# crowsonkb/k-diffusion

Measured on AMD Instinct MI355X. Metric: images/sec, 256x256 image_transformer_v2, 50-step DPM++2M (whole job), higher is better.
Workload: dtype f32

## Files before the change

k-diffusion_amd/csrc/gemm_x3.hip:

```cpp
#include "x3_common.h"

namespace kd {
namespace x3 {

struct XArgs {
  const float* A; const char* Wp; float* C;
  b16::u16* Cl; int c_split;
  const float* scale; int scale_stride, rows_per_sample; float eps;
  int M, N, n_tiles, n_splits;
  int n_heads; const float* qk_scale; const float* pos; const float* freq; int qkv_packed;
  float out_add;
  const float* sigma; float sigma_data; int gh, gw, chan;
  const float* R;
  int warm;
  unsigned long long* clk;
};

template <int NC , int EPI>
__global__ __launch_bounds__(256, NC <= 8 ? 2 : 1) void gemm_x3_astat_kernel(const XArgs p) {
  constexpr int K = NC * 16, NK = NC / 2;
  constexpr int NSTG = NC <= 8 ? 4 : 8, PDIST = NSTG - 1, PB = 4;
  constexpr bool GEGLU = EPI == KD_EPI_GEGLU;
  constexpr int NCOL = GEGLU ? 64 : 128;
  constexpr int NST = GEGLU ? 8 : 16;
  constexpr int WAREA = (NSTG / 4) * STG;
  constexpr int KH = WAREA / 128 >= K ? K : WAREA / 128;
  constexpr bool AG = NC >= 32;
  constexpr int NR = K / KH, CPR = KH / 4;
  constexpr int PIECES = 32 * CPR / 64;
  constexpr int SCL = K * 4 < 1024 ? 1024 : K * 4;
  static_assert(NK % NSTG == 0 || NSTG % NK == 0, "ring slot of a stage must be a compile-time constant");
  static_assert(CPR >= 16 && NC % NR == 0, "source-side chunk swizzle spans 16 chunk positions");
  extern __shared__ __attribute__((aligned(16))) char smem[];
  const int tid = threadIdx.x, lane = tid & 63, l31 = lane & 31, lh = lane >> 5;
  const int wid = __builtin_amdgcn_readfirstlane(tid >> 6);
  const auto warm = code_warm_begin<(NC <= 8 ? 14 : 24) * 1024>((int)blockIdx.x < p.warm && tid < 64);
  const PanelSplit ps = panel_split(p.n_splits, p.n_tiles);
  const int nt_begin = ps.t_begin, n_tiles = ps.t_end - ps.t_begin, total = n_tiles * NK;
  const int m0 = ps.panel * 128;
  const bool probe = p.clk && blockIdx.x == 0 && tid == 0;
  if (probe) { p.clk[0] = __builtin_amdgcn_s_memtime(); p.clk[1] = __builtin_amdgcn_s_memrealtime(); }
  const WgStamp wgs = wg_stamp_begin(p.clk);

  f32x16 acc[4];
  if constexpr (EPI == KD_EPI_RESIDUAL) {
    const int rrow = min(m0 + wid * 32 + l31, p.M - 1);
    const float* rp = p.R + (size_t)rrow * p.N + nt_begin * NCOL + 4 * lh;
#pragma unroll
    for (int j = 0; j < 4; ++j)
#pragma unroll
      for (int g = 0; g < 4; ++g) {
        const f32x4 v = *reinterpret_cast<const f32x4*>(rp + 32 * j + 8 * g);
#pragma unroll
        for (int e = 0; e < 4; ++e) acc[j][4 * g + e] = v[e];
      }
  }

  const char* wp = p.Wp + (size_t)nt_begin * NK * STG + wid * (PB * 1024) + lane * 16;
  auto issue_piece = [&](int s_, int j) {
    const int s = min(s_, total - 1);
    const char* src = wp + (size_t)s * STG;
    char* dst = smem + (s_ % NSTG) * STG + wid * (PB * 1024);
    __builtin_amdgcn_global_load_lds((const __attribute__((address_space(1))) void*)(src + j * 1024),
                                     (__attribute__((address_space(3))) void*)(dst + j * 1024), 16, 0, 0);
  };
  auto issue = [&](int s_) {
#pragma unroll
    for (int j = 0; j < PB; ++j) issue_piece(s_, j);
  };

  const int row = m0 + wid * 32 + l31;
  const bool ok = row < p.M;
  const int rowc = ok ? row : p.M - 1;
  bf16x8 a_hi[AG ? 1 : NC], a_lo[AG ? 1 : NC];
  float rs;
  {
    char* stage = smem + wid * WAREA;
    char* scl = smem + NSTG * STG + wid * SCL;
    const int r_first = min(m0 + wid * 32, p.M - 1), r_last = min(m0 + wid * 32 + 31, p.M - 1);
    constexpr bool nrm = EPI != KD_EPI_RESIDUAL;
    const bool uni = nrm && (p.scale_stride == 0 || r_first / p.rows_per_sample == r_last / p.rows_per_sample);
    if (uni) {
      const char* ssrc = reinterpret_cast<const char*>(p.scale + (size_t)(r_first / p.rows_per_sample) * p.scale_stride);
#pragma unroll
      for (int i = 0; i < SCL / 1024; ++i)
        __builtin_amdgcn_global_load_lds((const __attribute__((address_space(1))) void*)(ssrc + (i * 1024 + lane * 16) % (K * 4)),
                                         (__attribute__((address_space(3))) void*)(scl + i * 1024), 16, 0, 0);
    }
    const float* sp = p.scale + (size_t)(rowc / p.rows_per_sample) * p.scale_stride + 8 * lh;
    const float* spl = reinterpret_cast<const float*>(scl) + 8 * lh;
    float ssq = 0.f;
    static_for<NR>([&](auto r_) {
      constexpr int r = decltype(r_)::value;
#pragma unroll
      for (int i = 0; i < PIECES; ++i) {
        const int ci = i * 64 + lane, rr = ci / CPR, qs = ci % CPR;
        const int grow = min(m0 + wid * 32 + rr, p.M - 1);
        const char* src = reinterpret_cast<const char*>(p.A + (size_t)grow * K + r * KH) + ((qs ^ (rr & 15)) << 4);
        __builtin_amdgcn_global_load_lds((const __attribute__((address_space(1))) void*)src,
                                         (__attribute__((address_space(3))) void*)(stage + i * 1024), 16, 0, 0);
      }
// ... 20 lines not shown
        __builtin_amdgcn_sched_barrier(0);
        static_for<4>([&](auto u_) {
          constexpr int u = decltype(u_)::value;
#pragma unroll
          for (int e = 0; e < 4; ++e) ssq = fmaf(x0[u][e], x0[u][e], fmaf(x1[u][e], x1[u][e], ssq));
          u32x4 hi, lo;
          if constexpr (nrm) split8(x0[u] * s0[u], x1[u] * s1[u], hi, lo);
          else split8(x0[u], x1[u], hi, lo);
          if constexpr (AG) {
            areg_write4<8 * (c0 + u)>(hi);
            areg_write4<8 * (c0 + u) + 4>(lo);
          } else {
            asm volatile("" : "+v"(hi), "+v"(lo));
            a_hi[c0 + u] = __builtin_bit_cast(bf16x8, hi);
            a_lo[c0 + u] = __builtin_bit_cast(bf16x8, lo);
          }
        });
        __builtin_amdgcn_sched_barrier(0);
      });
      if constexpr (NR > 1) asm volatile("s_waitcnt lgkmcnt(0)" ::: "memory");
    });
    ssq += __shfl_xor(ssq, 32, 64);
    rs = nrm ? rsqrtf(ssq / (float)K + p.eps) : 1.f;
  }
  float py = 0.f, px = 0.f;
  if (EPI == KD_EPI_QKV) {
    qk_tab_fill(reinterpret_cast<float*>(smem + NSTG * STG + 4 * SCL + 4 * 2048), tid, p);
    token_pos(p.pos, rowc % p.rows_per_sample, py, px);
  }
  code_warm_end(warm);
  asm volatile("s_waitcnt vmcnt(0) lgkmcnt(0)" ::: "memory");
  KD_BARRIER();
  const bool full_panel = m0 + 128 <= p.M;
#pragma unroll
  for (int s = 0; s < PDIST; ++s) issue(s);
  if (probe) p.clk[4] = __builtin_amdgcn_s_memtime();

  const int o0 = swz64(l31, lh), o1 = swz64(l31, 2 + lh);
  char* strip = smem + NSTG * STG + 4 * SCL + wid * 2048;
  const char* qkc = smem + NSTG * STG + 4 * SCL + 4 * 2048;
  float* st_row[2];
  bool st_ok[2];
#pragma unroll
  for (int it = 0; it < 2; ++it) {
    const int r = m0 + wid * 32 + 16 * it + (lane >> 2);
    st_ok[it] = r < p.M;
    st_row[it] = p.C + (size_t)min(r, p.M - 1) * p.N + 4 * (lane & 3);
  }
  if constexpr (EPI != KD_EPI_RESIDUAL) {
#pragma unroll
    for (int j = 0; j < 4; ++j)
#pragma unroll
      for (int r = 0; r < 16; ++r) acc[j][r] = 0.f;
  }
  if constexpr (AG) asm volatile("s_nop 3" : "+v"(acc[0]), "+v"(acc[1]), "+v"(acc[2]), "+v"(acc[3]));

  bf16x8 wh[2][4], wl[2][4];
  int ou0[2] = {0, 0}, ou1[2] = {0, 0};
  if constexpr (EPI == KD_EPI_UNPATCH_NCHW) {
#pragma unroll
    for (int j = 0; j < 2; ++j) {
      const int np = 32 * j + l31, q = np >> 2, py = q / p.chan, cch = q - py * p.chan;
      const int n = np < 16 * p.chan ? (py * 4 + (np & 3)) * p.chan + cch : np;
      ou0[j] = swz64(n, lh);
      ou1[j] = swz64(n, 2 + lh);
    }
  }
  auto read_frags = [&](int slot, int h, bf16x8 (&fh)[4], bf16x8 (&fl)[4]) {
    if constexpr (EPI == KD_EPI_UNPATCH_NCHW) {
#pragma unroll
      for (int j = 0; j < 2; ++j) {
        const char* st = smem + slot * STG + (h ? ou1[j] : ou0[j]);
        fh[j] = *reinterpret_cast<const bf16x8*>(st);
        fl[j] = *reinterpret_cast<const bf16x8*>(st + IMG);
      }
    } else {
      const char* st = smem + slot * STG + (h ? o1 : o0);
#pragma unroll
      for (int j = 0; j < 4; ++j) {
        fh[j] = *reinterpret_cast<const bf16x8*>(st + j * 32 * 64);
        fl[j] = *reinterpret_cast<const bf16x8*>(st + IMG + j * 32 * 64);
      }
    }
  };
  wait_vm(PB * (PDIST - 1));
  KD_BARRIER();
  read_frags(0, 0, wh[0], wl[0]);

  for (int nt = 0; nt < n_tiles; ++nt) {
    static_for<NK>([&](auto ks_) {
      constexpr int ks = decltype(ks_)::value;
      const int s = nt * NK + ks;
      auto mm = [&](auto b_, int j, bool w_lo, auto a_lo_) {
        constexpr int b = decltype(b_)::value, al = decltype(a_lo_)::value, c = 2 * ks + b;
        if (EPI == KD_EPI_UNPATCH_NCHW && j >= 2) return;
        const bf16x8& w = w_lo ? wl[b][j] : wh[b][j];
        if constexpr (AG) mfma_ag<8 * c + 4 * al>(acc[j], w);
        else mfma_a(acc[j], w, al ? a_lo[c] : a_hi[c]);
      };
      constexpr std::integral_constant<int, 0> I0{};
      constexpr std::integral_constant<int, 1> I1{};
      if constexpr (AG) {
        mm(I0, 0, true, I0);
        __builtin_amdgcn_sched_barrier(0);
        read_frags(ks % NSTG, 1, wh[1], wl[1]);
        __builtin_amdgcn_sched_barrier(0);
#pragma unroll
        for (int j = 1; j < 4; ++j) mm(I0, j, true, I0);
      } else {
        read_frags(ks % NSTG, 1, wh[1], wl[1]);
#pragma unroll
        for (int j = 0; j < 4; ++j) mm(I0, j, true, I0);
      }
#pragma unroll
      for (int j = 0; j < 4; ++j) mm(I0, j, false, I1);
#pragma unroll
      for (int j = 0; j < 4; ++j) mm(I0, j, false, I0);
      if constexpr (!AG) {
        __builtin_amdgcn_sched_group_barrier(0x008, 1, 0);
        __builtin_amdgcn_sched_group_barrier(0x100, 8, 0);
        __builtin_amdgcn_sched_group_barrier(0x008, 11, 0);
      }
      __builtin_amdgcn_sched_barrier(0);
      {
        int allow = PB * (PDIST - 2);
        if (full_panel && nt > 0 && ks + 2 <= PDIST) allow += NST;
        wait_vm(allow);
        KD_BARRIER();
      }
      mm(I1, 0, true, I0);
      if constexpr (AG) __builtin_amdgcn_sched_barrier(0);
      read_frags((ks + 1) % NSTG, 0, wh[0], wl[0]);
      if constexpr (!AG) {
        __builtin_amdgcn_sched_group_barrier(0x008, 1, 0);
        __builtin_amdgcn_sched_group_barrier(0x100, 8, 0);
      }
      __builtin_amdgcn_sched_barrier(0);
      mm(I1, 1, true, I0);
      mm(I1, 2, true, I0);
      issue_piece(s + PDIST, 0);
      __builtin_amdgcn_sched_barrier(0);
      mm(I1, 3, true, I0);
      mm(I1, 0, false, I1);
      mm(I1, 1, false, I1);
      issue_piece(s + PDIST, 1);
      __builtin_amdgcn_sched_barrier(0);
      mm(I1, 2, false, I1);
      mm(I1, 3, false, I1);
      mm(I1, 0, false, I0);
      issue_piece(s + PDIST, 2);
      __builtin_amdgcn_sched_barrier(0);
      mm(I1, 1, false, I0);
      mm(I1, 2, false, I0);
      issue_piece(s + PDIST, 3);
      mm(I1, 3, false, I0);
      __builtin_amdgcn_sched_barrier(0);
    });
    if constexpr (AG) asm volatile("s_nop 15\n\ts_nop 3" : "+v"(acc[0]), "+v"(acc[1]), "+v"(acc[2]), "+v"(acc[3]));
    if (probe && nt == 0) p.clk[5] = __builtin_amdgcn_s_memtime();

    const int n0 = (nt_begin + nt) * NCOL;
    auto store_block = [&](const f32x4 (&v)[4], int col) {
#pragma unroll
      for (int hb = 0; hb < 2; ++hb) {
#pragma unroll
        for (int gg = 0; gg < 2; ++gg)
          *reinterpret_cast<f32x4*>(strip + l31 * 64 + (((2 * gg + lh) ^ ((l31 >> 2) & 1)) << 4)) = v[2 * hb + gg];
#pragma unroll
        for (int it = 0; it < 2; ++it) {
          const int r16 = 16 * it + (lane >> 2), c = lane & 3;
          const f32x4 o = *reinterpret_cast<const f32x4*>(strip + r16 * 64 + ((c ^ ((r16 >> 2) & 1)) << 4));
          if (st_ok[it]) st16(st_row[it] + col + 16 * hb, o);
        }
      }
    };
    if (GEGLU) {
      const float rsh = 0.5f * rs;
#pragma unroll
      for (int jj = 0; jj < 2; ++jj) {
        f32x4 blk[4];
#pragma unroll
        for (int g = 0; g < 4; ++g) {
          const f32x2 a = geglu_pair(f32x2{acc[2 * jj][4 * g], acc[2 * jj][4 * g + 1]} * rsh, f32x2{acc[2 * jj + 1][4 * g], acc[2 * jj + 1][4 * g + 1]} * rs);
          const f32x2 b = geglu_pair(f32x2{acc[2 * jj][4 * g + 2], acc[2 * jj][4 * g + 3]} * rsh, f32x2{acc[2 * jj + 1][4 * g + 2], acc[2 * jj + 1][4 * g + 3]} * rs);
          blk[g] = f32x4{a.x, a.y, b.x, b.y};
        }
        if (p.c_split) {
          float v[16], hi[16], lo[16];
#pragma unroll
          for (int g = 0; g < 4; ++g)
#pragma unroll
            for (int q = 0; q < 4; ++q) v[4 * g + q] = blk[g][q];
#pragma unroll
          for (int r = 0; r < 16; r += 2) {
            const unsigned h = pack_bf16(v[r], v[r + 1]);
            hi[r] = b16::bf_lo(h);
            hi[r + 1] = b16::bf_hi(h);
            lo[r] = v[r] - hi[r];
            lo[r + 1] = v[r + 1] - hi[r + 1];
          }
          const size_t off = (size_t)rowc * p.N + n0 + 32 * jj;
          b16::store_block_bf16(reinterpret_cast<b16::u16*>(p.C) + off, hi, lh, ok);
          b16::store_block_bf16(p.Cl + off, lo, lh, ok);
        } else {
          store_block(blk, n0 + 32 * jj);
        }
      }
    } else if (EPI == KD_EPI_QKV) {
#pragma unroll
      for (int vv = 0; vv < 2; ++vv) {
        const int vec = (n0 >> 6) + vv;
        const int which = vec >= 2 * p.n_heads ? 2 : (vec >= p.n_heads ? 1 : 0), head = vec - which * p.n_heads;
        f32x16& a0 = acc[2 * vv];
        f32x16& a1 = acc[2 * vv + 1];
        if (which < 2) {
          qk_prep_head(qkc, head, lh, a0, a1, rs, p.eps, py, px);
        } else {
#pragma unroll
          for (int r = 0; r < 16; ++r) { a0[r] *= rs; a1[r] *= rs; }
        }
#pragma unroll
        for (int jj = 0; jj < 2; ++jj) {
          f32x4 blk[4];
          const f32x16& a = jj ? a1 : a0;
          if (p.qkv_packed) {
#pragma unroll
            for (int g = 0; g < 4; ++g) blk[g] = pack_split4(f32x4{a[4 * g], a[4 * g + 1], a[4 * g + 2], a[4 * g + 3]});
          } else {
#pragma unroll
            for (int g = 0; g < 4; ++g) blk[g] = f32x4{a[4 * g], a[4 * g + 1], a[4 * g + 2], a[4 * g + 3]};
          }
          store_block(blk, n0 + 64 * vv + 32 * jj);
        }
      }
    } else if (EPI == KD_EPI_UNPATCH_NCHW) {
      const int per = p.gh * p.gw, bb = rowc / per, rr = rowc - bb * per, ty = rr / p.gw, tx = rr - ty * p.gw;
      float c_out = 1.f, c_skip = 0.f;
      if (p.sigma) {
        const float sg = p.sigma[bb], sd = p.sigma_data, var = sg * sg + sd * sd;
        c_skip = sd * sd / var;
        c_out = sg * sd / sqrtf(var);
      }
      const int Himg = 4 * p.gh, Wimg = 4 * p.gw;
#pragma unroll
      for (int j = 0; j < 2; ++j)
#pragma unroll
        for (int g = 0; g < 4; ++g) {
          const int q = 8 * j + 2 * g + lh, py = q / p.chan, cch = q - py * p.chan;
          if (q < 4 * p.chan && ok) {
            const size_t o = (((size_t)bb * p.chan + cch) * Himg + 4 * ty + py) * Wimg + 4 * tx;
            f32x4 v = f32x4{acc[j][4 * g], acc[j][4 * g + 1], acc[j][4 * g + 2], acc[j][4 * g + 3]} * (rs * c_out);
            if (p.sigma) v = v + *reinterpret_cast<const f32x4*>(p.R + o) * c_skip;
            st16(p.C + o, v);
          }
        }
    } else {
#pragma unroll
      for (int j = 0; j < 4; ++j) {
        f32x4 blk[4];
#pragma unroll
        for (int g = 0; g < 4; ++g) blk[g] = f32x4{acc[j][4 * g], acc[j][4 * g + 1], acc[j][4 * g + 2], acc[j][4 * g + 3]} * rs + p.out_add;
        store_block(blk, n0 + 32 * j);
      }
    }
    if (probe && nt == 0) p.clk[6] = __builtin_amdgcn_s_memtime();
#pragma unroll
    for (int j = 0; j < 4; ++j)
#pragma unroll
      for (int r = 0; r < 16; ++r) acc[j][r] = 0.f;
    if constexpr (AG) asm volatile("s_nop 3" : "+v"(acc[0]), "+v"(acc[1]), "+v"(acc[2]), "+v"(acc[3]));
  }
  asm volatile("s_waitcnt vmcnt(0)" ::: "memory");
  if (probe) { p.clk[2] = __builtin_amdgcn_s_memtime(); p.clk[3] = __builtin_amdgcn_s_memrealtime(); p.clk[7] = (unsigned long long)total; }
  wg_stamp_end(wgs);
}

template <int EPI>
__global__ __launch_bounds__(256, 2) void gemm_x3h_kernel(const XArgs p) {
  constexpr int NC = 16, K = 256, NK = 8;
  constexpr int NSTG = 4, PDIST = NSTG - 1, PB = 4, UNIT = 4;
  constexpr bool GEGLU = EPI == KD_EPI_GEGLU;
  constexpr int HCOL = GEGLU ? 32 : 64;
  constexpr int NST = GEGLU ? 4 : 8;
  constexpr int KH = 128, NR = K / KH, CPR = KH / 4, PIECES = 32 * CPR / 64, SCL = 1024, SUB = 8192, HALF = 4096, CB = 2;
  extern __shared__ __attribute__((aligned(16))) char smem[];
  const int tid = threadIdx.x, lane = tid & 63, l31 = lane & 31, lh = lane >> 5;
  const int wid = __builtin_amdgcn_readfirstlane(tid >> 6);
  const auto warm = code_warm_begin<20 * 1024>((int)blockIdx.x < p.warm && tid < 64);
  const PanelSplit ps = panel_split(p.n_splits, p.n_tiles);
  const int ht_begin = ps.t_begin, n_ht = ps.t_end - ps.t_begin, total = n_ht * UNIT;
  const int m0 = ps.panel * 128;
  const bool probe = p.clk && blockIdx.x == (gridDim.x * 5) / 8 && tid == 0;
  if (probe) { p.clk[0] = __builtin_amdgcn_s_memtime(); p.clk[1] = __builtin_amdgcn_s_memrealtime(); }
  const WgStamp wgs = wg_stamp_begin(p.clk);

  const char* wp = p.Wp + wid * 1024 + lane * 16;
  auto issue_piece = [&](int q_, int j) {
    const int q = min(q_, total - 1), ht = ht_begin + (q >> 2), u = q & 3;
    const char* src = wp + ((size_t)(ht >> 1) * NK + 2 * u + (j >> 1)) * STG + (j & 1) * IMG + (ht & 1) * HALF;
    char* dst = smem + (q_ % NSTG) * STG + (j >> 1) * SUB + (j & 1) * HALF + wid * 1024;
    __builtin_amdgcn_global_load_lds((const __attribute__((address_space(1))) void*)src, (__attribute__((address_space(3))) void*)dst, 16, 0, 0);
  };

  const int row = m0 + wid * 32 + l31;
  const bool ok = row < p.M;
  const int rowc = ok ? row : p.M - 1;
// ... 192 lines not shown
      }
#pragma unroll
      for (int jj = 0; jj < 2; ++jj) {
        f32x4 blk[4];
        const f32x16& a = acc[jj];
        if (p.qkv_packed) {
#pragma unroll
          for (int g = 0; g < 4; ++g) blk[g] = pack_split4(f32x4{a[4 * g], a[4 * g + 1], a[4 * g + 2], a[4 * g + 3]});
        } else {
#pragma unroll
          for (int g = 0; g < 4; ++g) blk[g] = f32x4{a[4 * g], a[4 * g + 1], a[4 * g + 2], a[4 * g + 3]};
        }
        store_block(blk, n0 + 32 * jj);
      }
    } else {
#pragma unroll
      for (int j = 0; j < 2; ++j) {
        f32x4 blk[4];
#pragma unroll
        for (int g = 0; g < 4; ++g) blk[g] = f32x4{acc[j][4 * g], acc[j][4 * g + 1], acc[j][4 * g + 2], acc[j][4 * g + 3]} * rs + p.out_add;
        store_block(blk, n0 + 32 * j);
      }
    }
    if (probe && h == 1) p.clk[10] = __builtin_amdgcn_s_memtime();
  }
  asm volatile("s_waitcnt vmcnt(0)" ::: "memory");
  if (probe) { p.clk[2] = __builtin_amdgcn_s_memtime(); p.clk[3] = __builtin_amdgcn_s_memrealtime(); p.clk[7] = (unsigned long long)total; }
  wg_stamp_end(wgs);
}

unsigned long long* g_clk = nullptr;


template <int NC, int EPI>
static int launch(const XArgs& a0, const char* nm, double flops, double bytes, hipStream_t s, int force_splits = 0) {
  constexpr int K = NC * 16, NSTG = NC <= 8 ? 4 : 8;
  constexpr int LDS = NSTG * STG + 4 * (K * 4 < 1024 ? 1024 : K * 4) + 4 * 2048 + 1024;
  const int panels = (a0.M + 127) / 128, best = best_n_splits(panels, a0.n_tiles, (NC <= 8 ? 2 : 1) * cu_count(), 1);
  const int forced = force_splits ? force_splits : opt(KD_OPT_x3_splits);
  XArgs a = a0;
  a.n_splits = forced > 0 && forced <= a0.n_tiles ? forced : best;
  const CfgName cfg(nm, "splits%d", a.n_splits);
  LaunchScope prof(cfg, flops, bytes, s);
  kd::launch<gemm_x3_astat_kernel<NC, EPI>>(dim3((unsigned)(panels * a.n_splits)), dim3(256), LDS, s, a);
  return check_launch("kd_gemm_f32(x3 astat)");
}

template <int EPI>
static int launch_half(const XArgs& a0, const char* nm, double flops, double bytes, hipStream_t s) {
  constexpr int LDS = 4 * STG + 4 * 1024 + 4 * 2048 + 1024;
  const int panels = (a0.M + 127) / 128, best = best_n_splits(panels, a0.n_tiles, 2 * cu_count(), 2);
  const int forced = opt(KD_OPT_x3_splits);
  XArgs a = a0;
  a.n_splits = forced > 0 && forced <= a0.n_tiles && a0.n_tiles % forced == 0 ? forced : best;
  const CfgName cfg(nm, "splits%d", a.n_splits);
  LaunchScope prof(cfg, flops, bytes, s);
  kd::launch<gemm_x3h_kernel<EPI>>(dim3((unsigned)(panels * a.n_splits)), dim3(256), LDS, s, a);
  return check_launch("kd_gemm_f32(x3 half tiles)");
}

}

int gemm_x3_try(const GemmP& d, hipStream_t s, int* rc) {
  using namespace x3;
  if (!opt(KD_OPT_x3)) return 1;
  if (d.precision != KD_PREC_SPLIT3 || d.a_mode != KD_A_PLAIN || !d.Wp || d.debug) return 1;
  const bool unpatch = d.epi == KD_EPI_UNPATCH_NCHW;
  if (unpatch && (d.K != 128 || !d.norm || d.ph != 4 || d.pw != 4 || d.N != 16 * d.chan || d.N > 64 || !opt(KD_OPT_x3_unpatch))) return 1;
  if (d.epi != KD_EPI_STORE && d.epi != KD_EPI_QKV && d.epi != KD_EPI_GEGLU && d.epi != KD_EPI_RESIDUAL && !unpatch) return 1;
  if (d.epi == KD_EPI_RESIDUAL ? (d.norm || !d.R || d.K != 512 || !opt(KD_OPT_x3_res)) : !d.norm) return 1;
  if (d.K != 128 && d.K != 256 && d.K != 512) return 1;
  const int ncol = d.epi == KD_EPI_GEGLU ? 64 : 128;
  if ((!unpatch && d.N % ncol) || d.M < opt(KD_OPT_x3_min_rows) || (d.norm && d.rows_per_sample <= 0)) return 1;
  if (d.epi == KD_EPI_QKV && (!d.rope_pos || !d.rope_freq || d.n_heads > 16)) return 1;
  if (d.c_split && (d.epi != KD_EPI_GEGLU || !d.C_lo || (d.N & 31))) return 1;
  XArgs a{};
  a.A = d.A; a.Wp = reinterpret_cast<const char*>(d.Wp); a.C = d.C;
// ... 36 lines not shown
```

k-diffusion_amd/csrc/gemm_x3r.hip:

```cpp
#include "x3_common.h"

namespace kd {
namespace x3 { extern unsigned long long* g_clk; }
namespace x3r {

using namespace x3;

constexpr int ASTG = 16384;
constexpr int STAGE = ASTG + STG;
constexpr int NSTG = 4, PDIST = NSTG - 1;

struct RArgs {
  const float* A; const char* Wp; float* C; const float* R;
  int M, N, K, nk;
  int gh, gw;
  const float* fac;
  int warm;
  unsigned long long* clk;
};

template <int AMODE, int EPI, bool LW, bool PROBE>
__global__ __launch_bounds__(LW ? 512 : 256, LW ? 2 : 1) void gemm_x3r_kernel(const RArgs p) {
  extern __shared__ __attribute__((aligned(16))) char smem[];
  const int tid = threadIdx.x, lane = tid & 63, l31 = lane & 31, lh = lane >> 5;
  const int wid_all = __builtin_amdgcn_readfirstlane(tid >> 6);
  const bool loader = LW && wid_all >= 4;
  const int wid = LW ? (wid_all & 3) : wid_all;
  const auto warm = code_warm_begin<12 * 1024>((int)blockIdx.x < p.warm && tid < 64);
  const int n_tiles = p.N / 128;
  const int tile = __builtin_amdgcn_readfirstlane(KD_XCD_CHUNK());
  const int nt = tile % n_tiles, mt = tile / n_tiles;
  const int m0 = mt * 128, n0 = nt * 128;
  const int nk = p.nk;
  const bool probe = PROBE && p.clk && blockIdx.x == (gridDim.x * 5) / 8 && tid == 0;
  if (probe) p.clk[13] = __builtin_amdgcn_s_memtime();
  const bool wide = PROBE && p.clk && p.clk[15] == 0x4b44ull && lane == 0;
  if (wide && wid_all == 0) p.clk[32 + 3 * blockIdx.x] = __builtin_amdgcn_s_memrealtime();

  f32x16 acc[4];
  const char* arow[4];
  const int Cin = p.K >> 2;
#pragma unroll
  for (int i = 0; i < 4; ++i) {
    const int rt = wid * 32 + 8 * i + (lane >> 3);
    const int q = (lane & 7) ^ ((rt >> 1) & 7);
    const int gm = min(m0 + rt, p.M - 1);
    if constexpr (AMODE == KD_A_MERGE2x2) {
      const int per = p.gh * p.gw, b = gm / per, rr = gm - b * per, ci = rr / p.gw, cj = rr - ci * p.gw;
      arow[i] = reinterpret_cast<const char*>(p.A + (((size_t)b * (2 * p.gh) + 2 * ci) * (2 * p.gw) + 2 * cj) * Cin) + q * 16;
    } else {
      arow[i] = reinterpret_cast<const char*>(p.A + (size_t)gm * p.K) + q * 16;
    }
  }
  const char* wp = p.Wp + (size_t)nt * nk * STG + wid * 4096 + lane * 16;
  auto issue = [&](int s_) {
// ... 173 lines not shown
    for (int j = 0; j < 4; ++j)
#pragma unroll
      for (int r = 0; r < 16; ++r) {
        const float skip = skp[j][r], diff = acc[j][r] - skip;
        acc[j][r] = (fabsf(fac) < 0.5f) ? skip + fac * diff : acc[j][r] - diff * (1.0f - fac);
      }
  }
#pragma unroll
  for (int j = 0; j < 4; ++j)
#pragma unroll
    for (int hb = 0; hb < 2; ++hb) {
#pragma unroll
      for (int gg = 0; gg < 2; ++gg) {
        const int g = 2 * hb + gg;
        *reinterpret_cast<f32x4*>(strip + l31 * 64 + (((2 * gg + lh) ^ ((l31 >> 2) & 1)) << 4)) =
            f32x4{acc[j][4 * g], acc[j][4 * g + 1], acc[j][4 * g + 2], acc[j][4 * g + 3]};
      }
#pragma unroll
      for (int it = 0; it < 2; ++it) {
        const int r16 = 16 * it + (lane >> 2), cc = lane & 3;
        const f32x4 o = *reinterpret_cast<const f32x4*>(strip + r16 * 64 + ((cc ^ ((r16 >> 2) & 1)) << 4));
        if (st_ok[it]) st16(st_row[it] + 32 * j + 16 * hb, o);
      }
    }
  if (probe) { asm volatile("s_waitcnt vmcnt(0)" ::: "memory"); p.clk[14] = __builtin_amdgcn_s_memtime(); }
  if (wide && wid_all == 0) { asm volatile("s_waitcnt vmcnt(0)" ::: "memory"); p.clk[32 + 3 * blockIdx.x + 1] = __builtin_amdgcn_s_memrealtime(); }
}

template <int AMODE, int EPI, bool LW, bool PROBE>
static int launch_lw(const RArgs& a, const char* nm, double flops, double bytes, hipStream_t s) {
  constexpr int LDS = NSTG * STAGE + 4 * 2048;
  const long tiles = (long)((a.M + 127) / 128) * (a.N / 128);
  LaunchScope prof(nm, flops, bytes, s);
  kd::launch<gemm_x3r_kernel<AMODE, EPI, LW, PROBE>>(dim3((unsigned)tiles), dim3(LW ? 512 : 256), LDS, s, a);
  return check_launch("kd_gemm_f32(x3 residual / merge)");
}
template <int AMODE, int EPI>
static int launch(const RArgs& a, const char* nm, double flops, double bytes, hipStream_t s) {
  if (a.clk) return opt(KD_OPT_x3r_lw) ? launch_lw<AMODE, EPI, true, true>(a, nm, flops, bytes, s) : launch_lw<AMODE, EPI, false, true>(a, nm, flops, bytes, s);
  return opt(KD_OPT_x3r_lw) ? launch_lw<AMODE, EPI, true, false>(a, nm, flops, bytes, s) : launch_lw<AMODE, EPI, false, false>(a, nm, flops, bytes, s);
}

}

int gemm_x3r_try(const GemmP& d, hipStream_t s, int* rc) {
  using namespace x3r;
  const int mode = opt(KD_OPT_x3r);
  if (!mode) return 1;
  if (d.precision != KD_PREC_SPLIT3 || d.norm || !d.Wp || d.debug || d.a_split || d.c_split) return 1;
  if (d.a_mode != KD_A_PLAIN && d.a_mode != KD_A_MERGE2x2) return 1;
  if (d.epi != KD_EPI_STORE && d.epi != KD_EPI_RESIDUAL && d.epi != KD_EPI_SPLIT_LERP) return 1;
  if (d.epi == KD_EPI_SPLIT_LERP && (d.a_mode != KD_A_PLAIN || !d.R || !d.fac || ((d.N >> 2) & 127) || d.gh <= 0 || d.gw <= 0 || d.M % (d.gh * d.gw) || !opt(KD_OPT_x3r_split)))
    return 1;
  if ((d.K & 31) || (d.N & 127) || d.M < opt(KD_OPT_x3r_min_rows) || d.out_add != 0.f) return 1;
  if (mode != 2 && d.K < 256) return 1;
  if (d.a_mode == KD_A_MERGE2x2 && ((d.K >> 2) & 31)) return 1;
  RArgs a{};
  a.A = d.A; a.Wp = reinterpret_cast<const char*>(d.Wp); a.C = d.C; a.R = d.R;
  a.M = d.M; a.N = d.N; a.K = d.K; a.nk = d.K / 32; a.gh = d.gh; a.gw = d.gw; a.fac = d.fac;
  a.warm = d.warm;
  a.clk = x3::g_clk;
  const double flops = 2.0 * d.M * (double)d.N * d.K;
  const double bytes = 4.0 * ((double)d.M * d.K + (double)d.N * d.K + (double)d.M * d.N * (d.epi == KD_EPI_STORE ? 1 : 2));
  const ProfName nm("gemm_x3r", "gemm_x3r<a%d,e%d> M=%d N=%d K=%d", d.a_mode, d.epi, d.M, d.N, d.K);
  if (d.a_mode == KD_A_PLAIN && d.epi == KD_EPI_RESIDUAL) *rc = launch<KD_A_PLAIN, KD_EPI_RESIDUAL>(a, nm, flops, bytes, s);
  else if (d.epi == KD_EPI_SPLIT_LERP) *rc = launch<KD_A_PLAIN, KD_EPI_SPLIT_LERP>(a, nm, flops, bytes, s);
  else if (d.a_mode == KD_A_PLAIN) *rc = launch<KD_A_PLAIN, KD_EPI_STORE>(a, nm, flops, bytes, s);
// ... 9 lines not shown
```

Measured before the change: 231.6.

## Specialize large-K GEMM kernel for full panels, static LDS slots, and zero-init MFMA

For the NC>=32 (AG) GEMM path, the tile loop becomes a lambda templated on full-panel and later-tile flags. Full panels drop row-bounds checks on stores and use compile-time waitcnt immediates. Weight prefetch goes through a new issue_piece_sb helper with constant ring slots and register-held offsets. Accumulator zeroing is replaced by a zero-init MFMA variant on the first k-step, and timing probes are compiled out unless a clk buffer is present. The aim is to cut scalar and vector overhead and register pressure in the hot loop, at the cost of more template instantiations and larger code, which is why the code-warm size is raised.

```diff
diff --git a/k-diffusion_amd/csrc/gemm_x3.hip b/k-diffusion_amd/csrc/gemm_x3.hip
--- a/k-diffusion_amd/csrc/gemm_x3.hip
+++ b/k-diffusion_amd/csrc/gemm_x3.hip
@@ -16,7 +16,8 @@
   unsigned long long* clk;
 };
 
-template <int NC , int EPI>
+template <int NC , int EPI,
+          bool PROBE = false >
 __global__ __launch_bounds__(256, NC <= 8 ? 2 : 1) void gemm_x3_astat_kernel(const XArgs p) {
   constexpr int K = NC * 16, NK = NC / 2;
   constexpr int NSTG = NC <= 8 ? 4 : 8, PDIST = NSTG - 1, PB = 4;
@@ -26,6 +27,8 @@
   constexpr int WAREA = (NSTG / 4) * STG;
   constexpr int KH = WAREA / 128 >= K ? K : WAREA / 128;
   constexpr bool AG = NC >= 32;
+  constexpr bool PR = PROBE || !AG;
+  constexpr bool ZC = AG && EPI != KD_EPI_RESIDUAL;
   constexpr int NR = K / KH, CPR = KH / 4;
   constexpr int PIECES = 32 * CPR / 64;
   constexpr int SCL = K * 4 < 1024 ? 1024 : K * 4;
@@ -34,11 +37,11 @@
   extern __shared__ __attribute__((aligned(16))) char smem[];
   const int tid = threadIdx.x, lane = tid & 63, l31 = lane & 31, lh = lane >> 5;
   const int wid = __builtin_amdgcn_readfirstlane(tid >> 6);
-  const auto warm = code_warm_begin<(NC <= 8 ? 14 : 24) * 1024>((int)blockIdx.x < p.warm && tid < 64);
+  const auto warm = code_warm_begin<(NC <= 8 ? 14 : NC >= 32 ? 32 : 24) * 1024>((int)blockIdx.x < p.warm && tid < 64);
   const PanelSplit ps = panel_split(p.n_splits, p.n_tiles);
   const int nt_begin = ps.t_begin, n_tiles = ps.t_end - ps.t_begin, total = n_tiles * NK;
   const int m0 = ps.panel * 128;
-  const bool probe = p.clk && blockIdx.x == 0 && tid == 0;
+  const bool probe = PR && p.clk && blockIdx.x == 0 && tid == 0;
   if (probe) { p.clk[0] = __builtin_amdgcn_s_memtime(); p.clk[1] = __builtin_amdgcn_s_memrealtime(); }
   const WgStamp wgs = wg_stamp_begin(p.clk);
 
@@ -67,6 +70,14 @@
   auto issue = [&](int s_) {
 #pragma unroll
     for (int j = 0; j < PB; ++j) issue_piece(s_, j);
+  };
+  unsigned voff[PB];
+  const char* wbase = p.Wp + (size_t)nt_begin * NK * STG;
+  auto issue_piece_sb = [&](int s_, auto slot_, auto j_) {
+    constexpr int slot = decltype(slot_)::value, j = decltype(j_)::value;
+    const int s = min(s_, total - 1);
+    asm volatile("" : "+v"(voff[j]));
+    b16::glds16(wbase + (size_t)s * STG + voff[j], smem + slot * STG + wid * (PB * 1024) + j * 1024);
   };
 
   const int row = m0 + wid * 32 + l31;
@@ -153,9 +164,15 @@
   asm volatile("s_waitcnt vmcnt(0) lgkmcnt(0)" ::: "memory");
   KD_BARRIER();
   const bool full_panel = m0 + 128 <= p.M;
-#pragma unroll
-  for (int s = 0; s < PDIST; ++s) issue(s);
-  if (probe) p.clk[4] = __builtin_amdgcn_s_memtime();
+  if constexpr (AG) {
+#pragma unroll
+    for (int j = 0; j < PB; ++j) voff[j] = wid * (PB * 1024) + j * 1024 + lane * 16;
+    static_for<PDIST>([&](auto s_) { static_for<PB>([&](auto j_) { issue_piece_sb(decltype(s_)::value, s_, j_); }); });
+  } else {
+#pragma unroll
+    for (int s = 0; s < PDIST; ++s) issue(s);
+  }
+  if constexpr (PR) { if (probe) p.clk[4] = __builtin_amdgcn_s_memtime(); }
 
   const int o0 = swz64(l31, lh), o1 = swz64(l31, 2 + lh);
   char* strip = smem + NSTG * STG + 4 * SCL + wid * 2048;
@@ -168,13 +185,13 @@
     st_ok[it] = r < p.M;
     st_row[it] = p.C + (size_t)min(r, p.M - 1) * p.N + 4 * (lane & 3);
   }
-  if constexpr (EPI != KD_EPI_RESIDUAL) {
+  if constexpr (EPI != KD_EPI_RESIDUAL && !ZC) {
 #pragma unroll
     for (int j = 0; j < 4; ++j)
 #pragma unroll
       for (int r = 0; r < 16; ++r) acc[j][r] = 0.f;
   }
-  if constexpr (AG) asm volatile("s_nop 3" : "+v"(acc[0]), "+v"(acc[1]), "+v"(acc[2]), "+v"(acc[3]));
+  if constexpr (AG && !ZC) asm volatile("s_nop 3" : "+v"(acc[0]), "+v"(acc[1]), "+v"(acc[2]), "+v"(acc[3]));
 
   bf16x8 wh[2][4], wl[2][4];
   int ou0[2] = {0, 0}, ou1[2] = {0, 0};
@@ -208,7 +225,8 @@
   KD_BARRIER();
   read_frags(0, 0, wh[0], wl[0]);
 
-  for (int nt = 0; nt < n_tiles; ++nt) {
+  auto tile = [&](const int nt, auto full_, auto later_) {
+    constexpr bool FULL = decltype(full_)::value, LATER = decltype(later_)::value;
     static_for<NK>([&](auto ks_) {
       constexpr int ks = decltype(ks_)::value;
       const int s = nt * NK + ks;
@@ -216,11 +234,20 @@
         constexpr int b = decltype(b_)::value, al = decltype(a_lo_)::value, c = 2 * ks + b;
         if (EPI == KD_EPI_UNPATCH_NCHW && j >= 2) return;
         const bf16x8& w = w_lo ? wl[b][j] : wh[b][j];
-        if constexpr (AG) mfma_ag<8 * c + 4 * al>(acc[j], w);
+        if constexpr (ZC && c == 0 && al == 0) {
+          if (w_lo) mfma_ag0<0>(acc[j], w);
+          else mfma_ag<0>(acc[j], w);
+        } else if constexpr (AG) mfma_ag<8 * c + 4 * al>(acc[j], w);
         else mfma_a(acc[j], w, al ? a_lo[c] : a_hi[c]);
+      };
+      auto request = [&](auto j_) {
+        if constexpr (AG) issue_piece_sb(s + PDIST, std::integral_constant<int, (ks + PDIST) % NSTG>{}, j_);
+        else issue_piece(s + PDIST, decltype(j_)::value);
       };
       constexpr std::integral_constant<int, 0> I0{};
       constexpr std::integral_constant<int, 1> I1{};
+      constexpr std::integral_constant<int, 2> I2{};
+      constexpr std::integral_constant<int, 3> I3{};
       if constexpr (AG) {
         mm(I0, 0, true, I0);
         __builtin_amdgcn_sched_barrier(0);
@@ -244,9 +271,13 @@
       }
       __builtin_amdgcn_sched_barrier(0);
       {
-        int allow = PB * (PDIST - 2);
-        if (full_panel && nt > 0 && ks + 2 <= PDIST) allow += NST;
-        wait_vm(allow);
+        if constexpr (AG) {
+          asm volatile("s_waitcnt vmcnt(%0)" :: "n"(PB * (PDIST - 2) + (FULL && LATER && ks + 2 <= PDIST ? NST : 0)) : "memory");
+        } else {
+          int allow = PB * (PDIST - 2);
+          if (full_panel && nt > 0 && ks + 2 <= PDIST) allow += NST;
+          wait_vm(allow);
+        }
         KD_BARRIER();
       }
       mm(I1, 0, true, I0);
@@ -259,26 +290,26 @@
       __builtin_amdgcn_sched_barrier(0);
       mm(I1, 1, true, I0);
       mm(I1, 2, true, I0);
-      issue_piece(s + PDIST, 0);
+      request(I0);
       __builtin_amdgcn_sched_barrier(0);
       mm(I1, 3, true, I0);
       mm(I1, 0, false, I1);
       mm(I1, 1, false, I1);
-      issue_piece(s + PDIST, 1);
+      request(I1);
       __builtin_amdgcn_sched_barrier(0);
       mm(I1, 2, false, I1);
       mm(I1, 3, false, I1);
       mm(I1, 0, false, I0);
-      issue_piece(s + PDIST, 2);
+      request(I2);
       __builtin_amdgcn_sched_barrier(0);
       mm(I1, 1, false, I0);
       mm(I1, 2, false, I0);
-      issue_piece(s + PDIST, 3);
+      request(I3);
       mm(I1, 3, false, I0);
       __builtin_amdgcn_sched_barrier(0);
     });
     if constexpr (AG) asm volatile("s_nop 15\n\ts_nop 3" : "+v"(acc[0]), "+v"(acc[1]), "+v"(acc[2]), "+v"(acc[3]));
-    if (probe && nt == 0) p.clk[5] = __builtin_amdgcn_s_memtime();
+    if constexpr (PR) { if (probe && nt == 0) p.clk[5] = __builtin_amdgcn_s_memtime(); }
 
     const int n0 = (nt_begin + nt) * NCOL;
     auto store_block = [&](const f32x4 (&v)[4], int col) {
@@ -291,7 +322,7 @@
         for (int it = 0; it < 2; ++it) {
           const int r16 = 16 * it + (lane >> 2), c = lane & 3;
           const f32x4 o = *reinterpret_cast<const f32x4*>(strip + r16 * 64 + ((c ^ ((r16 >> 2) & 1)) << 4));
-          if (st_ok[it]) st16(st_row[it] + col + 16 * hb, o);
+          if (FULL || st_ok[it]) st16(st_row[it] + col + 16 * hb, o);
         }
       }
     };
@@ -321,8 +352,8 @@
             lo[r + 1] = v[r + 1] - hi[r + 1];
           }
           const size_t off = (size_t)rowc * p.N + n0 + 32 * jj;
-          b16::store_block_bf16(reinterpret_cast<b16::u16*>(p.C) + off, hi, lh, ok);
-          b16::store_block_bf16(p.Cl + off, lo, lh, ok);
+          b16::store_block_bf16(reinterpret_cast<b16::u16*>(p.C) + off, hi, lh, FULL || ok);
+          b16::store_block_bf16(p.Cl + off, lo, lh, FULL || ok);
         } else {
           store_block(blk, n0 + 32 * jj);
         }
@@ -384,15 +415,33 @@
         store_block(blk, n0 + 32 * j);
       }
     }
-    if (probe && nt == 0) p.clk[6] = __builtin_amdgcn_s_memtime();
-#pragma unroll
-    for (int j = 0; j < 4; ++j)
-#pragma unroll
-      for (int r = 0; r < 16; ++r) acc[j][r] = 0.f;
-    if constexpr (AG) asm volatile("s_nop 3" : "+v"(acc[0]), "+v"(acc[1]), "+v"(acc[2]), "+v"(acc[3]));
+    if constexpr (PR) { if (probe && nt == 0) p.clk[6] = __builtin_amdgcn_s_memtime(); }
+    if constexpr (!ZC) {
+#pragma unroll
+      for (int j = 0; j < 4; ++j)
+#pragma unroll
+        for (int r = 0; r < 16; ++r) acc[j][r] = 0.f;
+      if constexpr (AG) asm volatile("s_nop 3" : "+v"(acc[0]), "+v"(acc[1]), "+v"(acc[2]), "+v"(acc[3]));
+    }
+  };
+  constexpr std::false_type NO{};
+  constexpr std::true_type YES{};
+  if constexpr (AG) {
+    if (full_panel) {
+      tile(0, YES, NO);
+      if constexpr (EPI != KD_EPI_RESIDUAL) {
+        for (int nt = 1; nt < n_tiles; ++nt) tile(nt, YES, YES);
+      }
+    } else {
+      for (int nt = 0; nt < (EPI == KD_EPI_RESIDUAL ? 1 : n_tiles); ++nt) tile(nt, NO, NO);
+    }
+  } else {
+    for (int nt = 0; nt < n_tiles; ++nt) tile(nt, NO, NO);
   }
   asm volatile("s_waitcnt vmcnt(0)" ::: "memory");
-  if (probe) { p.clk[2] = __builtin_amdgcn_s_memtime(); p.clk[3] = __builtin_amdgcn_s_memrealtime(); p.clk[7] = (unsigned long long)total; }
+  if constexpr (PR) {
+    if (probe) { p.clk[2] = __builtin_amdgcn_s_memtime(); p.clk[3] = __builtin_amdgcn_s_memrealtime(); p.clk[7] = (unsigned long long)total; }
+  }
   wg_stamp_end(wgs);
 }
 
@@ -651,8 +700,9 @@
 unsigned long long* g_clk = nullptr;
 
 
-template <int NC, int EPI>
+template <int NC, int EPI, bool PROBE = false>
 static int launch(const XArgs& a0, const char* nm, double flops, double bytes, hipStream_t s, int force_splits = 0) {
+  if constexpr (NC >= 32 && !PROBE) { if (a0.clk) return launch<NC, EPI, true>(a0, nm, flops, bytes, s, force_splits); }
   constexpr int K = NC * 16, NSTG = NC <= 8 ? 4 : 8;
   constexpr int LDS = NSTG * STG + 4 * (K * 4 < 1024 ? 1024 : K * 4) + 4 * 2048 + 1024;
   const int panels = (a0.M + 127) / 128, best = best_n_splits(panels, a0.n_tiles, (NC <= 8 ? 2 : 1) * cu_count(), 1);
@@ -661,7 +711,7 @@
   a.n_splits = forced > 0 && forced <= a0.n_tiles ? forced : best;
   const CfgName cfg(nm, "splits%d", a.n_splits);
   LaunchScope prof(cfg, flops, bytes, s);
-  kd::launch<gemm_x3_astat_kernel<NC, EPI>>(dim3((unsigned)(panels * a.n_splits)), dim3(256), LDS, s, a);
+  kd::launch<gemm_x3_astat_kernel<NC, EPI, PROBE>>(dim3((unsigned)(panels * a.n_splits)), dim3(256), LDS, s, a);
   return check_launch("kd_gemm_f32(x3 astat)");
 }
 
```

After: 231.8, median of 2. About the same (+0.1%).

## Rewrite x3r residual/merge GEMM around 16x16x32 bf16 MFMA fragments

Applied to the files above, without the earlier changes.

Adds a new main loop for the store/residual x3r GEMM that uses 16x16x32 bf16 MFMA instructions instead of the previous 32x32 variant. It brings new swizzled LDS layouts for A, W and the output strip, and software-pipelines the split of f32 activations into hi/lo bf16 across stages, interleaved with the MFMAs. The old 32-wide kernel is kept only for the split+lerp epilogue. The aim is better MFMA issue and LDS access patterns, at the cost of more fragment bookkeeping and a new swizzle scheme whose packed weight layout must match the existing packer.

```diff
diff --git a/k-diffusion_amd/csrc/gemm_x3r.hip b/k-diffusion_amd/csrc/gemm_x3r.hip
--- a/k-diffusion_amd/csrc/gemm_x3r.hip
+++ b/k-diffusion_amd/csrc/gemm_x3r.hip
@@ -1,4 +1,5 @@
 #include "x3_common.h"
+#include "x3_mfma16.h"
 
 namespace kd {
 namespace x3 { extern unsigned long long* g_clk; }
@@ -21,6 +22,213 @@
 
 template <int AMODE, int EPI, bool LW, bool PROBE>
 __global__ __launch_bounds__(LW ? 512 : 256, LW ? 2 : 1) void gemm_x3r_kernel(const RArgs p) {
+  static_assert(EPI == KD_EPI_STORE || EPI == KD_EPI_RESIDUAL, "the token split + lerp runs on gemm_x3r_split32_kernel");
+  extern __shared__ __attribute__((aligned(16))) char smem[];
+  const int tid = threadIdx.x, lane = tid & 63, l15 = lane & 15, lq = lane >> 4;
+  const int wid_all = __builtin_amdgcn_readfirstlane(tid >> 6);
+  const bool loader = LW && wid_all >= 4;
+  const int wid = LW ? (wid_all & 3) : wid_all;
+  const auto warm = code_warm_begin<12 * 1024>((int)blockIdx.x < p.warm && tid < 64);
+  const int n_tiles = p.N / 128;
+  const int tile = __builtin_amdgcn_readfirstlane(KD_XCD_CHUNK());
+  const int nt = tile % n_tiles, mt = tile / n_tiles;
+  const int m0 = mt * 128, n0 = nt * 128;
+  const int nk = p.nk;
+  const bool probe = PROBE && p.clk && blockIdx.x == (gridDim.x * 5) / 8 && tid == 0;
+  if (probe) p.clk[13] = __builtin_amdgcn_s_memtime();
+  const bool wide = PROBE && p.clk && p.clk[15] == 0x4b44ull && lane == 0;
+  if (wide && wid_all == 0) p.clk[32 + 3 * blockIdx.x] = __builtin_amdgcn_s_memrealtime();
+
+  f32x4 acc[2][8];
+  const char* arow[4];
+  const int Cin = p.K >> 2;
+#pragma unroll
+  for (int i = 0; i < 4; ++i) {
+    const int rt = wid * 32 + 8 * i + (lane >> 3);
+    const int q = m16::a_pos(rt, lane & 7);
+    const int gm = min(m0 + rt, p.M - 1);
+    if constexpr (AMODE == KD_A_MERGE2x2) {
+      const int per = p.gh * p.gw, b = gm / per, rr = gm - b * per, ci = rr / p.gw, cj = rr - ci * p.gw;
+      arow[i] = reinterpret_cast<const char*>(p.A + (((size_t)b * (2 * p.gh) + 2 * ci) * (2 * p.gw) + 2 * cj) * Cin) + q * 16;
+    } else {
+      arow[i] = reinterpret_cast<const char*>(p.A + (size_t)gm * p.K) + q * 16;
+    }
+  }
+  const char* wp = p.Wp + (size_t)nt * nk * STG + wid * 4096 + m16::w_src_off(lane * 16);
+  auto issue_one = [&](int s_, int i) {
+    const int s = min(s_, nk - 1);
+    char* slot = smem + (s_ % NSTG) * STAGE;
+    if (i < 4) {
+      size_t aoff;
+      if constexpr (AMODE == KD_A_MERGE2x2) {
+        const int k0 = s * 32, quad = k0 / Cin, e = k0 - quad * Cin;
+        aoff = ((size_t)(quad >> 1) * (2 * p.gw) + (quad & 1)) * Cin * 4 + (size_t)e * 4;
+      } else {
+        aoff = (size_t)s * 128;
+      }
+      __builtin_amdgcn_global_load_lds((const __attribute__((address_space(1))) void*)(arow[i] + aoff),
+                                       (__attribute__((address_space(3))) void*)(slot + wid * 4096 + i * 1024), 16, 0, 0);
+    } else {
+      __builtin_amdgcn_global_load_lds((const __attribute__((address_space(1))) void*)(wp + (size_t)s * STG + (i - 4) * 1024),
+                                       (__attribute__((address_space(3))) void*)(slot + ASTG + wid * 4096 + (i - 4) * 1024), 16, 0, 0);
+    }
+  };
+  auto issue = [&](int s_) {
+#pragma unroll
+    for (int i = 0; i < 8; ++i) issue_one(s_, i);
+  };
+  if constexpr (LW) {
+    if (loader) {
+#pragma unroll
+      for (int s = 0; s < PDIST; ++s) issue(s);
+      wait_vm(8 * (PDIST - 1));
+      KD_BARRIER();
+      for (int s = 0; s < nk; ++s) {
+        wait_vm(8 * (PDIST - 2));
+        KD_BARRIER();
+        issue(s + PDIST);
+      }
+      asm volatile("s_waitcnt vmcnt(0)" ::: "memory");
+      if (wide && wid_all == 4) p.clk[32 + 3 * blockIdx.x + 2] = __builtin_amdgcn_s_memrealtime();
+      return;
+    }
+  } else {
+#pragma unroll
+    for (int s = 0; s < PDIST; ++s) issue(s);
+  }
+  auto out_row = [&](int gm) -> size_t { return (size_t)gm * p.N + n0; };
+#pragma unroll
+  for (int g = 0; g < 2; ++g) {
+    const int rrow = min(m0 + wid * 32 + 16 * g + l15, p.M - 1);
+    if constexpr (EPI == KD_EPI_RESIDUAL) {
+      const float* rp = p.R + out_row(rrow) + 4 * lq;
+#pragma unroll
+      for (int blk = 0; blk < 8; ++blk) acc[g][blk] = *reinterpret_cast<const f32x4*>(rp + 16 * blk);
+    } else {
+#pragma unroll
+      for (int blk = 0; blk < 8; ++blk) acc[g][blk] = f32x4{0.f, 0.f, 0.f, 0.f};
+    }
+  }
+
+#pragma unroll
+  for (int g = 0; g < 2; ++g)
+#pragma unroll
+    for (int blk = 0; blk < 8; ++blk) asm volatile("" : "+v"(acc[g][blk]));
+  code_warm_end(warm);
+
+  const int a0 = m16::a_frag_off(wid * 32, lane, 0);
+  const int w0 = m16::w_frag_off(0, lane);
+  f32x4 xr[2][2];
+  bf16x8 wh[2][4], wl[2][4];
+  u32x4 ahu[2][2], alu[2][2];
+  auto read_a = [&](int slot, auto I) {
+    constexpr int i = decltype(I)::value, g = i >> 1, e = i & 1;
+    xr[g][e] = *reinterpret_cast<const f32x4*>(smem + slot * STAGE + ((a0 + 2048 * g) ^ (16 * e)));
+  };
+  auto read_w = [&](int slot, auto HF, auto R) {
+    constexpr int hf = decltype(HF)::value, r = decltype(R)::value, bi = r >> 1;
+    const char* wst = smem + slot * STAGE + ASTG + w0 + (4 * hf + bi) * 1024;
+    if constexpr ((r & 1) == 0) wh[hf][bi] = *reinterpret_cast<const bf16x8*>(wst);
+    else wl[hf][bi] = *reinterpret_cast<const bf16x8*>(wst + IMG);
+  };
+  unsigned sp_h;
+  float sp_a, sp_b;
+  auto split_step = [&](auto PAR, auto PC, auto ST) {
+    constexpr int par = decltype(PAR)::value, pc = decltype(PC)::value, st = decltype(ST)::value, g = pc >> 2, q = pc & 3;
+    const float a = xr[g][q >> 1][2 * (q & 1)], b = xr[g][q >> 1][2 * (q & 1) + 1];
+    if constexpr (st == 0) {
+      sp_h = pack_bf16(a, b);
+      asm volatile("" : "+v"(sp_h));
+      sp_a = b16::bf_lo(sp_h);
+      asm volatile("" : "+v"(sp_a));
+    } else if constexpr (st == 1) {
+      sp_a = a - sp_a;
+      sp_b = b16::bf_hi(sp_h);
+      asm volatile("" : "+v"(sp_a), "+v"(sp_b));
+    } else {
+      unsigned l = pack_bf16(sp_a, b - sp_b);
+      asm volatile("" : "+v"(l));
+      ahu[par][g][q] = sp_h;
+      alu[par][g][q] = l;
+    }
+  };
+  auto mm = [&](auto PAR, auto M) {
+    constexpr int par = decltype(PAR)::value, m = decltype(M)::value, hf = m / 24, t = (m % 24) / 8, bi = (m % 8) / 2, g = m & 1;
+    const bf16x8 a = __builtin_bit_cast(bf16x8, t == 1 ? alu[par][g] : ahu[par][g]);
+    acc[g][4 * hf + bi] = __builtin_amdgcn_mfma_f32_16x16x32_bf16(t == 0 ? wl[hf][bi] : wh[hf][bi], a, acc[g][4 * hf + bi], 0, 0, 0);
+  };
+  using std::integral_constant;
+#define KD_GAP() __builtin_amdgcn_sched_barrier(0)
+  auto stage = [&](auto PAR, int s) {
+    constexpr int par = decltype(PAR)::value;
+    const int slot = s % NSTG, nslot = (s + 1) % NSTG;
+    if (PROBE && par == 0 && probe && s == 8) p.clk[8] = __builtin_amdgcn_s_memtime();
+    static_for<48>([&](auto M) {
+      constexpr int m = decltype(M)::value;
+      if constexpr (m == 12) {
+        if (PROBE && par == 0 && probe && s == 8) p.clk[9] = __builtin_amdgcn_s_memtime();
+        if constexpr (!LW) wait_vm(8 * (PDIST - 2));
+        if (PROBE && par == 0 && probe && s == 8) p.clk[10] = __builtin_amdgcn_s_memtime();
+        KD_BARRIER();
+        if (PROBE && par == 0 && probe && s == 8) p.clk[11] = __builtin_amdgcn_s_memtime();
+      }
+      mm(PAR, M);
+      if constexpr (m < 8) read_w(slot, integral_constant<int, 1>{}, M);
+      else if constexpr (m >= 12 && m < 16) read_a(nslot, integral_constant<int, m - 12>{});
+      else if constexpr (m >= 16 && m < 40)
+        split_step(integral_constant<int, par ^ 1>{}, integral_constant<int, (m - 16) / 3>{}, integral_constant<int, (m - 16) % 3>{});
+      else if constexpr (m >= 40) read_w(nslot, integral_constant<int, 0>{}, integral_constant<int, m - 40>{});
+      if constexpr (!LW && m >= 12 && m < 20) issue_one(s + PDIST, m - 12);
+      KD_GAP();
+    });
+    if (PROBE && par == 0 && probe && s == 8) p.clk[12] = __builtin_amdgcn_s_memtime();
+  };
+  if constexpr (!LW) wait_vm(8 * (PDIST - 1));
+  KD_BARRIER();
+  static_for<4>([&](auto I) { read_a(0, I); });
+  static_for<8>([&](auto R) { read_w(0, integral_constant<int, 0>{}, R); });
+  static_for<8>([&](auto PC) {
+    static_for<3>([&](auto ST) { split_step(integral_constant<int, 0>{}, PC, ST); });
+  });
+  if (probe) { p.clk[0] = __builtin_amdgcn_s_memtime(); p.clk[1] = __builtin_amdgcn_s_memrealtime(); }
+  {
+    int s = 0;
+    for (; s + 1 < nk; s += 2) {
+      stage(integral_constant<int, 0>{}, s);
+      stage(integral_constant<int, 1>{}, s + 1);
+    }
+    if (s < nk) stage(integral_constant<int, 0>{}, s);
+  }
+#undef KD_GAP
+  if (probe) { p.clk[2] = __builtin_amdgcn_s_memtime(); p.clk[3] = __builtin_amdgcn_s_memrealtime(); p.clk[7] = (unsigned long long)nk; }
+  if constexpr (!LW) asm volatile("s_waitcnt vmcnt(0)" ::: "memory");
+
+  char* strip = smem + NSTG * STAGE + wid * 2048;
+  float* st_row[2];
+  bool st_ok[2];
+#pragma unroll
+  for (int it = 0; it < 2; ++it) {
+    const int r = m0 + wid * 32 + 16 * it + (lane >> 2);
+    st_ok[it] = r < p.M;
+    st_row[it] = p.C + out_row(min(r, p.M - 1)) + 4 * (lane & 3);
+  }
+#pragma unroll
+  for (int blk = 0; blk < 8; ++blk) {
+#pragma unroll
+    for (int g = 0; g < 2; ++g) *reinterpret_cast<f32x4*>(strip + m16::strip_off(16 * g + l15, lq)) = acc[g][blk];
+#pragma unroll
+    for (int it = 0; it < 2; ++it) {
+      const f32x4 o = *reinterpret_cast<const f32x4*>(strip + m16::strip_off(16 * it + (lane >> 2), lane & 3));
+      if (st_ok[it]) st16(st_row[it] + 16 * blk, o);
+    }
+  }
+  if (probe) { asm volatile("s_waitcnt vmcnt(0)" ::: "memory"); p.clk[14] = __builtin_amdgcn_s_memtime(); }
+  if (wide && wid_all == 0) { asm volatile("s_waitcnt vmcnt(0)" ::: "memory"); p.clk[32 + 3 * blockIdx.x + 1] = __builtin_amdgcn_s_memrealtime(); }
+}
+
+template <bool LW, bool PROBE>
+__global__ __launch_bounds__(LW ? 512 : 256, LW ? 2 : 1) void gemm_x3r_split32_kernel(const RArgs p) {
+  constexpr int AMODE = KD_A_PLAIN, EPI = KD_EPI_SPLIT_LERP;
   extern __shared__ __attribute__((aligned(16))) char smem[];
   const int tid = threadIdx.x, lane = tid & 63, l31 = lane & 31, lh = lane >> 5;
   const int wid_all = __builtin_amdgcn_readfirstlane(tid >> 6);
@@ -260,7 +468,8 @@
   constexpr int LDS = NSTG * STAGE + 4 * 2048;
   const long tiles = (long)((a.M + 127) / 128) * (a.N / 128);
   LaunchScope prof(nm, flops, bytes, s);
-  kd::launch<gemm_x3r_kernel<AMODE, EPI, LW, PROBE>>(dim3((unsigned)tiles), dim3(LW ? 512 : 256), LDS, s, a);
+  if constexpr (EPI == KD_EPI_SPLIT_LERP) kd::launch<gemm_x3r_split32_kernel<LW, PROBE>>(dim3((unsigned)tiles), dim3(LW ? 512 : 256), LDS, s, a);
+  else kd::launch<gemm_x3r_kernel<AMODE, EPI, LW, PROBE>>(dim3((unsigned)tiles), dim3(LW ? 512 : 256), LDS, s, a);
   return check_launch("kd_gemm_f32(x3 residual / merge)");
 }
 template <int AMODE, int EPI>
diff --git a/k-diffusion_amd/csrc/x3_mfma16.h b/k-diffusion_amd/csrc/x3_mfma16.h
--- /dev/null
+++ b/k-diffusion_amd/csrc/x3_mfma16.h
@@ -0,0 +1,29 @@
+#pragma once
+#ifdef __HIPCC__
+#include <hip/hip_runtime.h>
+#define KD_M16 __host__ __device__ __forceinline__
+#else
+#define KD_M16 inline
+#endif
+
+namespace kd {
+namespace m16 {
+
+KD_M16 int a_pos(int row, int ch) { return ch ^ (((row >> 1) + 2) & 7); }
+KD_M16 int a_off(int row, int ch) { return row * 128 + (a_pos(row, ch) << 4); }
+KD_M16 int a_frag_off(int r0, int lane, int e) { return a_off(r0 + (lane & 15), 2 * (lane >> 4) + e); }
+
+KD_M16 int w_pos(int row, int ch) { return ch ^ ((0 - (row >> 2)) & 3); }
+KD_M16 int w_off(int row, int ch) { return row * 64 + (w_pos(row, ch) << 4); }
+KD_M16 int w_frag_off(int blk, int lane) { return w_off(16 * blk + (lane & 15), lane >> 4); }
+KD_M16 int w_packed_pos(int row, int ch) { return ch ^ ((row >> 2) & 3); }
+KD_M16 int w_src_off(int lds_off) {
+  const int row = lds_off >> 6, pos = (lds_off >> 4) & 3;
+  const int ch = w_pos(row, pos);
+  return row * 64 + (w_packed_pos(row, ch) << 4);
+}
+
+KD_M16 int strip_off(int row, int ch) { return row * 64 + ((ch ^ ((row >> 1) & 3)) << 4); }
+
+}
+}
```

Result: no change. 229.5 before, 231.4 after, median of 6 (+0.8%).
